# SamsungLabs/cloud_transformers

Hardware: AMD Instinct MI355X
Metric: points/sec fwd+bwd MHCT, 4096-pt batch, 1/2/4/8 MI355X; % HBM roofline (higher is better)
Workload: dtype f32; 1 GPU; north-star op-level: B=8 clouds x N=4096 pts, H=64 heads, C=16 feat/head, 2D grid W=32, reduce=max, keys=tanh(randn), seed 1234+rank; step = Splat fwd, Slice fwd, Slice bwd, Splat bwd (key cotangents summed); per_gpu_batch=8, parallelism=replica-sharded clouds x1 (no collective), world_size_seen=1, hip_graph=True, steps_per_graph=10

## Files before the change

### cloud_transformers_amd/csrc/ct_raster_bwd_fused.h

```cpp
#pragma once

template <bool HAS_PAD, int WT, int NT = 0, int CT = 0>
__global__ void __launch_bounds__(kSortThreads) slice_splat_bwd_kernel(RasterArgs a_arg, GridW<2> g_arg) {
  const GridW<2> g = grid2_of<WT>(g_arg);
  RasterArgs a = a_arg;
  if constexpr (NT > 0) a.N = NT;
  if constexpr (CT > 0) a.C = CT;
  extern __shared__ __align__(16) unsigned char lds_raw[];
  const int G = WT ? WT * WT : g.G, W1 = WT ? WT : g.W[1], N = a.N, C = a.C;
  const SortLds L = sort_lds(G, N, C);
  float4* T4 = (float4*)(lds_raw + L.tile);
  int* acc = (int*)(lds_raw + L.acc);
  float4* ZG = (float4*)(lds_raw + L.tile);
  float4* Sg = (float4*)(lds_raw + L.stage);
  const float2* AB = (const float2*)(lds_raw + L.ab);
  unsigned* s_max = (unsigned*)(lds_raw + L.misc);
  unsigned* s_k = s_max + C;
  int* s_tie = (int*)(s_k + 1);
  const int b = blockIdx.z;
  const size_t bh = (size_t)b * a.H + blockIdx.y;
  const int tid = threadIdx.x;
  const int off[4] = {0, W1, 1, W1 + 1};
  const bool has = (tid << 2) < N;
  const int n0 = has ? (tid << 2) : 0;
  const int ngroups = C >> 2;
  const float* const feat = a.tile_in2;

  float gq[4][4];
  float fq[4][4];
  float cvq[4];
  const float* const src0 = a.src + bh * C * (size_t)N;
  const float* const fea0 = feat + bh * C * (size_t)N;
  const float* const cnv0 = a.tile_in + bh * C * (size_t)G;
  const unsigned ln0 = (unsigned)n0, lc0 = (unsigned)(tid < G ? tid : 0);
  auto request1 = [&](int grp, int cj) {
    const float4 t = ld_stream4(src0 + (size_t)(grp * 4 + cj) * N + ln0);
    gq[cj][0] = t.x; gq[cj][1] = t.y; gq[cj][2] = t.z; gq[cj][3] = t.w;
    cvq[cj] = ld_stream(cnv0 + (size_t)(grp * 4 + cj) * G + lc0);
  };
  auto request_feat1 = [&](int grp, int cj) {
    const float4 t = ld_stream4(fea0 + (size_t)(grp * 4 + cj) * N + ln0);
    fq[cj][0] = t.x; fq[cj][1] = t.y; fq[cj][2] = t.z; fq[cj][3] = t.w;
  };
  PlaneKeys PK;
  load_plane_keys(a, g, W1, bh, PK);
  SortedPlane S;
  float pv[4];
#pragma unroll
  for (int i = 0; i < 4; ++i) pv[i] = (HAS_PAD && has) ? ct_load_pad(a.pad, a.pad_dtype, (size_t)b * N + n0 + i) : 1.0f;

  sort_plane(a, PK, G, W1, sort_ptrs(lds_raw, L, C), C, S, nullptr, [&]() {
#pragma unroll
    for (int cj = 0; cj < 4; ++cj) request1(0, cj);
  });
  for (int i = tid; i < G; i += kSortThreads) ((int4*)acc)[i] = make_int4(0, 0, 0, 0);
  if (tid == 0) Sg[N] = make_float4(0.0f, 0.0f, 0.0f, 0.0f);
  if (tid < 4) s_tie[tid] = 0;
  const float Kf = (float)(*s_k);

  float gsx[2][kItemLen], gsy[2][kItemLen];
#pragma unroll
  for (int u = 0; u < 2; ++u)
#pragma unroll
    for (int j = 0; j < kItemLen; ++j) gsx[u][j] = gsy[u][j] = 0.0f;
  float gs[4][2];
#pragma unroll
  for (int i = 0; i < 4; ++i) gs[i][0] = gs[i][1] = 0.0f;
  unsigned long long tied = 0ull;

  const float* const key0 = a.pos.keys + bh * 2 * (size_t)N;

  auto group = [&](const int grp, auto more) {
    const int ch0 = grp * 4;
    asm volatile("" : "+v"(S.rk01), "+v"(S.rk23));
#pragma unroll
    for (int cj = 0; cj < 4; ++cj) {
      float m = 0.0f;
#pragma unroll
      for (int i = 0; i < 4; ++i) {
        float x = HAS_PAD ? gq[cj][i] * pv[i] : gq[cj][i];
        x = has ? x : 0.0f;
        gq[cj][i] = x;
        x = fabsf(x);
        m = fmaxf(m, (x < __builtin_inff()) ? x : __builtin_inff());
      }
      const unsigned mb = wave_max_u32(__float_as_uint(m));
      if ((tid & 63) == 0) atomicMax(&s_max[ch0 + cj], mb);
    }
    if (has) {
      const unsigned rk[4] = {S.rk01 & kRankMask, (S.rk01 >> 16) & kRankMask, S.rk23 & kRankMask, (S.rk23 >> 16) & kRankMask};
#pragma unroll
      for (int i = 0; i < 4; ++i) Sg[rk[i]] = make_float4(gq[0][i], gq[1][i], gq[2][i], gq[3][i]);
    }
    if (tid < G) T4[tid] = make_float4(cvq[0], cvq[1], cvq[2], cvq[3]);
    __syncthreads();

    float iq[4];
    bool any_float = false;
#pragma unroll
    for (int cj = 0; cj < 4; ++cj) {
      float q;
      bool fixed;
      fx_quantum(__uint_as_float(s_max[ch0 + cj]) * Kf, q, iq[cj], fixed);
      if (!fixed) {
        iq[cj] = 0.0f;
        any_float = true;
      }
      iq[cj] = __uint_as_float(__builtin_amdgcn_readfirstlane(__float_as_uint(iq[cj])));
    }
    auto item = [&](auto U) {
      constexpr int u = decltype(U)::value;
      const int Y = S.cell[u] < 0 ? 0 : S.cell[u];
      asm volatile("" : "+v"(S.ent8[u][0]), "+v"(S.ent8[u][1]));
      float4 cv[4];
#pragma unroll
      for (int v = 0; v < 4; ++v) cv[v] = T4[Y + off[v]];
      float4 xn = *(const float4*)((const unsigned char*)Sg + 2u * CT_E8(S, u, 0));
      float2 wn = *(const float2*)((const unsigned char*)AB + CT_E8(S, u, 0));
      ct_f2 s01[4], s23[4];
#pragma unroll
      for (int v = 0; v < 4; ++v) s01[v] = s23[v] = ct_f2{0.0f, 0.0f};
#pragma unroll
      for (int j = 0; j < kItemLen; ++j) {
        if constexpr (u == 0) request_feat1(grp, j);
        const float4 x = xn;
        const float2 wf = wn;
        if (j + 1 < kItemLen) {
          xn = *(const float4*)((const unsigned char*)Sg + 2u * CT_E8(S, u, j + 1));
          wn = *(const float2*)((const unsigned char*)AB + CT_E8(S, u, j + 1));
        }
        const ct_f2 x01 = {x.x, x.y}, x23 = {x.z, x.w};
        const float w1x = wf.x, w1y = wf.y, w0x = 1.0f - w1x, w0y = 1.0f - w1y;
        const float cw[4] = {w0x * w0y, w1x * w0y, w0x * w1y, w1x * w1y};
        float gw[4];
#pragma unroll
        for (int v = 0; v < 4; ++v) {
          const ct_f2 cwv = {cw[v], cw[v]};
          s01[v] = __builtin_elementwise_fma(x01, cwv, s01[v]);
          s23[v] = __builtin_elementwise_fma(x23, cwv, s23[v]);
          const ct_f2 c01 = {cv[v].x, cv[v].y}, c23 = {cv[v].z, cv[v].w};
          const ct_f2 pr = __builtin_elementwise_fma(c23, x23, c01 * x01);
          gw[v] = pr.x + pr.y;
        }
        gsx[u][j] = __builtin_fmaf(gw[3] - gw[2], w1y, __builtin_fmaf(gw[1] - gw[0], w0y, gsx[u][j]));
        gsy[u][j] = __builtin_fmaf(gw[3] - gw[1], w1x, __builtin_fmaf(gw[2] - gw[0], w0x, gsy[u][j]));
        asm volatile("" : "+v"(gsx[u][j]), "+v"(gsy[u][j]));
        CT_SB;
      }
      if (S.cell[u] >= 0) {
        const ct_f2 iq01 = {iq[0], iq[1]}, iq23 = {iq[2], iq[3]};
        int* Tc = acc + Y;
#pragma unroll
        for (int v = 0; v < 4; ++v) {
          const ct_f2 a01 = s01[v] * iq01, a23 = s23[v] * iq23;
          atomicAdd(Tc + off[v], cvt_rpi(a01.x));
          atomicAdd(Tc + G + off[v], cvt_rpi(a01.y));
          atomicAdd(Tc + 2 * G + off[v], cvt_rpi(a23.x));
          atomicAdd(Tc + 3 * G + off[v], cvt_rpi(a23.y));
        }
      }
      CT_SB;
    };
    item(std::integral_constant<int, 0>{});
    if (S.cell[1] >= 0) item(std::integral_constant<int, 1>{});
    if (any_float) {
#pragma unroll 1
      for (int cj = 0; cj < 4; ++cj)
        if (iq[cj] == 0.0f) scatter_float_channel<HAS_PAD>(a, g, bh, b, ch0 + cj, (float*)(acc + cj * G), 1, 0);
    }
    const float4 tx = *(const float4*)(key0 + ln0), ty = *(const float4*)(key0 + N + ln0);
    __syncthreads();

    float4 zc = make_float4(0.0f, 0.0f, 0.0f, 0.0f);
    float gv[4] = {0.0f, 0.0f, 0.0f, 0.0f};
    if (tid < G) {
      zc = T4[tid];
      float* gout = a.tile_out + (bh * C + ch0) * (size_t)G + tid;
#pragma unroll
      for (int cj = 0; cj < 4; ++cj) {
        float q, iqd;
        bool fixed;
        fx_quantum(__uint_as_float(s_max[ch0 + cj]) * Kf, q, iqd, fixed);
        const int r = acc[cj * G + tid];
        gv[cj] = fixed ? (float)r * q : __int_as_float(r);
        __builtin_nontemporal_store(gv[cj], gout + (size_t)cj * G);
      }
    }
    const unsigned zw[4] = {__float_as_uint(zc.x), __float_as_uint(zc.y), __float_as_uint(zc.z), __float_as_uint(zc.w)};
    {
      int nzt = 0;
#pragma unroll
      for (int k = 0; k < 4; ++k) nzt += (zw[k] != 0u);
      nzt = wave_sum_i32(nzt);
      if ((tid & 63) == 0 && nzt) atomicAdd(&s_tie[(grp & 1) * 2], nzt);
    }
    __syncthreads();
    if (tid < G) {
      ZG[tid] = make_float4(__uint_as_float(zw[0] ? zw[0] : kNoMatch), __uint_as_float(zw[1] ? zw[1] : kNoMatch), gv[0], gv[1]);
      ZG[G + tid] = make_float4(__uint_as_float(zw[2] ? zw[2] : kNoMatch), __uint_as_float(zw[3] ? zw[3] : kNoMatch), gv[2], gv[3]);
    }
    __syncthreads();

    int nm = 0;
    if (has) {
      float kx[4] = {tx.x, tx.y, tx.z, tx.w}, ky[4] = {ty.x, ty.y, ty.z, ty.w};
#pragma unroll
      for (int i = 0; i < 4; ++i) {
        if constexpr (decltype(more)::value) request1(grp + 1, i);
        asm volatile("" : "+v"(kx[i]), "+v"(ky[i]));
        Pt2 p;
        pt2_from_keys(kx[i], ky[i], g, W1, p);
        float gw[4] = {0.0f, 0.0f, 0.0f, 0.0f};
#pragma unroll
        for (int pr = 0; pr < 2; ++pr) {
          const float4* Zp = ZG + (size_t)pr * G + p.base;
          const float xa = HAS_PAD ? fq[2 * pr][i] * pv[i] : fq[2 * pr][i];
          const float xb = HAS_PAD ? fq[2 * pr + 1][i] * pv[i] : fq[2 * pr + 1][i];
          ct_f4 zg[4];
#pragma unroll
          for (int v = 0; v < 4; ++v) zg[v] = *(const ct_f4*)(Zp + off[v]);
#pragma unroll
          for (int v = 0; v < 4; ++v) asm volatile("" : "+v"(zg[v].x), "+v"(zg[v].y), "+v"(zg[v].z), "+v"(zg[v].w));
          float gfa = 0.0f, gfb = 0.0f;
#pragma unroll
          for (int v = 0; v < 4; ++v) {
            const unsigned ba = __float_as_uint(xa * p.cw[v]), bb = __float_as_uint(xb * p.cw[v]);
            const bool ma = ba == __float_as_uint(zg[v].x), mb = bb == __float_as_uint(zg[v].y);
            nm += (int)ma;
            nm += (int)mb;
            asm volatile("" : "+v"(nm));
            const float ga = ma ? zg[v].z : 0.0f, gb = mb ? zg[v].w : 0.0f;
            gfa = __builtin_fmaf(ga, p.cw[v], gfa);
            gfb = __builtin_fmaf(gb, p.cw[v], gfb);
            gw[v] = __builtin_fmaf(gb, xb, __builtin_fmaf(ga, xa, gw[v]));
          }
          fq[2 * pr][i] = HAS_PAD ? gfa * pv[i] : gfa;
          fq[2 * pr + 1][i] = HAS_PAD ? gfb * pv[i] : gfb;
        }
        gs[i][0] = __builtin_fmaf(gw[3] - gw[2], p.w1y, __builtin_fmaf(gw[1] - gw[0], p.w0y, gs[i][0]));
        gs[i][1] = __builtin_fmaf(gw[3] - gw[1], p.w1x, __builtin_fmaf(gw[2] - gw[0], p.w0x, gs[i][1]));
        asm volatile("" : "+v"(gs[i][0]), "+v"(gs[i][1]), "+v"(fq[0][i]), "+v"(fq[1][i]), "+v"(fq[2][i]), "+v"(fq[3][i]));
        __builtin_amdgcn_sched_barrier(0);
      }
#pragma unroll
      for (int cj = 0; cj < 4; ++cj)
        st_stream4(a.dst + (bh * C + ch0 + cj) * (size_t)N + n0, make_float4(fq[cj][0], fq[cj][1], fq[cj][2], fq[cj][3]));
    } else if constexpr (decltype(more)::value) {
#pragma unroll
      for (int cj = 0; cj < 4; ++cj) request1(grp + 1, cj);
    }
    nm = wave_sum_i32(nm);
    if ((tid & 63) == 0 && nm) atomicAdd(&s_tie[(grp & 1) * 2 + 1], nm);
    __syncthreads();
    const int* tw = s_tie + (grp & 1) * 2;
    if (tw[0] != tw[1]) tied |= 1ull << grp;
    if (tid < 2) s_tie[((grp & 1) ^ 1) * 2 + tid] = 0;
    if (tid < G) ((int4*)acc)[tid] = make_int4(0, 0, 0, 0);
  };
  int grp = 0;
  for (; grp + 1 < ngroups; ++grp) group(grp, std::true_type{});
  group(grp, std::false_type{});

  if (tied != 0ull) {
    __builtin_amdgcn_fence(__ATOMIC_RELEASE, "workgroup");
    asm volatile("s_waitcnt vmcnt(0)" ::: "memory");
    __syncthreads();
    __builtin_amdgcn_fence(__ATOMIC_ACQUIRE, "workgroup");
    RasterArgs a2 = a;
    a2.src = feat;
    PtRows R;
    R.Nr = N; R.so = 0; R.wt = false;
    for (int gi = 0; gi < ngroups; ++gi) {
      if (!((tied >> gi) & 1ull)) continue;
      const int cabs = gi << 2;
      const float* zin = a.tile_in + (bh * C + cabs) * (size_t)G;
      const float* gin = a.tile_out + (bh * C + cabs) * (size_t)G;
      __syncthreads();
      {
        int nz_unused = 0;
        unsigned long long nzp_unused = 0ull;
        unsigned xzp_unused = 0u;
        stage_tile_pairs<false>(ZG, zin, gin, 2, G, nz_unused, nzp_unused, xzp_unused);
      }
      __syncthreads();
      if (has) {
        const float4 tx = *(const float4*)(key0 + ln0), ty = *(const float4*)(key0 + N + ln0);
        const float kx[4] = {tx.x, tx.y, tx.z, tx.w}, ky[4] = {ty.x, ty.y, ty.z, ty.w};
        int nm_unused = 0;
        unsigned u0 = 0u, u1 = 0u;
        splat_bwd_quad<HAS_PAD, true, WT, true>(a2, g, ZG, bh, b, cabs, 4, n0, R, kx, ky, gs, nm_unused, u0, u1, false);
      }
    }
    __syncthreads();
  }

  float2* Gs = (float2*)Sg;
#pragma unroll
  for (int u = 0; u < 2; ++u)
#pragma unroll
    for (int j = 0; j < kItemLen; ++j)
      *(float2*)((unsigned char*)Gs + CT_E8(S, u, j)) = make_float2(gsx[u][j], gsy[u][j]);
  __syncthreads();
  if (has) {
    const unsigned rw[4] = {S.rk01 & 0xffffu, S.rk01 >> 16, S.rk23 & 0xffffu, S.rk23 >> 16};
    float2 gk[4];
#pragma unroll
    for (int i = 0; i < 4; ++i) {
      gk[i] = Gs[rw[i] & kRankMask];
      gk[i].x *= (rw[i] & kInsideX) ? 1.0f : 0.0f;
      gk[i].y *= (rw[i] & kInsideY) ? 1.0f : 0.0f;
    }
    if (a.fold_gpos != nullptr) {
      st_stream4(a.fold_gpos + (bh * 2 + 0) * N + n0, make_float4(gk[0].x, gk[1].x, gk[2].x, gk[3].x));
      st_stream4(a.fold_gpos + (bh * 2 + 1) * N + n0, make_float4(gk[0].y, gk[1].y, gk[2].y, gk[3].y));
    }
    const float4 tx = *(const float4*)(key0 + ln0), ty = *(const float4*)(key0 + N + ln0);
    float4 ox = make_float4(gs[0][0] * ct_key_mask(tx.x), gs[1][0] * ct_key_mask(tx.y), gs[2][0] * ct_key_mask(tx.z), gs[3][0] * ct_key_mask(tx.w));
    float4 oy = make_float4(gs[0][1] * ct_key_mask(ty.x), gs[1][1] * ct_key_mask(ty.y), gs[2][1] * ct_key_mask(ty.z), gs[3][1] * ct_key_mask(ty.w));
    ox.x += gk[0].x; ox.y += gk[1].x; ox.z += gk[2].x; ox.w += gk[3].x;
    oy.x += gk[0].y; oy.y += gk[1].y; oy.z += gk[2].y; oy.w += gk[3].y;
    *(float4*)(a.g_pos + (bh * 2 + 0) * N + n0) = ox;
    *(float4*)(a.g_pos + (bh * 2 + 1) * N + n0) = oy;
  }
}
```

Measured before the change: 193.9 million points/s.

## Use buffer-resource streaming loads and reuse sorted-plane weights instead of reloading keys

Replaces the global streaming loads and stores of point, cell and feature rows with raw buffer loads and stores that use a per-block resource descriptor and scalar row offsets. This is meant to cut 64-bit address arithmetic and VGPR use. The per-group reload of point keys and the pt2_from_keys recomputation are replaced by reading bilinear weights from the sorted AB LDS table plus base cells stashed in LDS. The final key mask comes from the inside bits in the rank words rather than a key reload. This trades global key traffic and ALU work for extra LDS reads, and it assumes the per-plane data fits in 32-bit buffer offsets.

```diff
diff --git a/cloud_transformers_amd/csrc/ct_raster_bwd_fused.h b/cloud_transformers_amd/csrc/ct_raster_bwd_fused.h
--- a/cloud_transformers_amd/csrc/ct_raster_bwd_fused.h
+++ b/cloud_transformers_amd/csrc/ct_raster_bwd_fused.h
@@ -1,4 +1,29 @@
 #pragma once
+
+typedef unsigned ct_u4 __attribute__((ext_vector_type(4)));
+struct StreamBuf {
+  __amdgpu_buffer_rsrc_t r;
+};
+constexpr int kBufNt = 2;
+__device__ __forceinline__ StreamBuf stream_buf(const float* base, unsigned bytes) {
+  StreamBuf b;
+  b.r = __builtin_amdgcn_make_buffer_rsrc((void*)base, 0, (int)bytes, 0x00020000);
+  return b;
+}
+__device__ __forceinline__ float4 buf_ld_stream4(const StreamBuf& b, unsigned voff, unsigned soff) {
+  const ct_u4 v = __builtin_amdgcn_raw_buffer_load_b128(b.r, (int)voff, (int)soff, kBufNt);
+  return make_float4(__uint_as_float(v.x), __uint_as_float(v.y), __uint_as_float(v.z), __uint_as_float(v.w));
+}
+__device__ __forceinline__ float buf_ld_stream(const StreamBuf& b, unsigned voff, unsigned soff) {
+  return __uint_as_float(__builtin_amdgcn_raw_buffer_load_b32(b.r, (int)voff, (int)soff, kBufNt));
+}
+__device__ __forceinline__ void buf_st_stream4(const StreamBuf& b, unsigned voff, unsigned soff, float4 v) {
+  const ct_u4 t = {__float_as_uint(v.x), __float_as_uint(v.y), __float_as_uint(v.z), __float_as_uint(v.w)};
+  __builtin_amdgcn_raw_buffer_store_b128(t, b.r, (int)voff, (int)soff, kBufNt);
+}
+__device__ __forceinline__ void buf_st_stream(const StreamBuf& b, unsigned voff, unsigned soff, float v) {
+  __builtin_amdgcn_raw_buffer_store_b32(__float_as_uint(v), b.r, (int)voff, (int)soff, kBufNt);
+}
 
 template <bool HAS_PAD, int WT, int NT = 0, int CT = 0>
 __global__ void __launch_bounds__(kSortThreads) slice_splat_bwd_kernel(RasterArgs a_arg, GridW<2> g_arg) {
@@ -29,17 +54,21 @@
   float gq[4][4];
   float fq[4][4];
   float cvq[4];
-  const float* const src0 = a.src + bh * C * (size_t)N;
-  const float* const fea0 = feat + bh * C * (size_t)N;
-  const float* const cnv0 = a.tile_in + bh * C * (size_t)G;
-  const unsigned ln0 = (unsigned)n0, lc0 = (unsigned)(tid < G ? tid : 0);
+  const unsigned ln0 = (unsigned)n0;
+  const unsigned pt_row = (unsigned)N * 4u, cell_row = (unsigned)G * 4u;
+  const StreamBuf b_src = stream_buf(a.src + bh * C * (size_t)N, (unsigned)C * pt_row);
+  const StreamBuf b_fea = stream_buf(feat + bh * C * (size_t)N, (unsigned)C * pt_row);
+  const StreamBuf b_dst = stream_buf(a.dst + bh * C * (size_t)N, (unsigned)C * pt_row);
+  const StreamBuf b_cnv = stream_buf(a.tile_in + bh * C * (size_t)G, (unsigned)C * cell_row);
+  const StreamBuf b_gz = stream_buf(a.tile_out + bh * C * (size_t)G, (unsigned)C * cell_row);
+  const unsigned vo_pt = ln0 * 4u, vo_cell = tid < G ? (unsigned)tid * 4u : 0u;
   auto request1 = [&](int grp, int cj) {
-    const float4 t = ld_stream4(src0 + (size_t)(grp * 4 + cj) * N + ln0);
+    const float4 t = buf_ld_stream4(b_src, vo_pt, (unsigned)(grp * 4 + cj) * pt_row);
     gq[cj][0] = t.x; gq[cj][1] = t.y; gq[cj][2] = t.z; gq[cj][3] = t.w;
-    cvq[cj] = ld_stream(cnv0 + (size_t)(grp * 4 + cj) * G + lc0);
+    cvq[cj] = buf_ld_stream(b_cnv, vo_cell, (unsigned)(grp * 4 + cj) * cell_row);
   };
   auto request_feat1 = [&](int grp, int cj) {
-    const float4 t = ld_stream4(fea0 + (size_t)(grp * 4 + cj) * N + ln0);
+    const float4 t = buf_ld_stream4(b_fea, vo_pt, (unsigned)(grp * 4 + cj) * pt_row);
     fq[cj][0] = t.x; fq[cj][1] = t.y; fq[cj][2] = t.z; fq[cj][3] = t.w;
   };
   PlaneKeys PK;
@@ -53,6 +82,8 @@
 #pragma unroll
     for (int cj = 0; cj < 4; ++cj) request1(0, cj);
   });
+  uint2* const s_cell = (uint2*)(lds_raw + L.mark);
+  s_cell[tid] = make_uint2((unsigned)PK.base[0] | (unsigned)PK.base[1] << 16, (unsigned)PK.base[2] | (unsigned)PK.base[3] << 16);
   for (int i = tid; i < G; i += kSortThreads) ((int4*)acc)[i] = make_int4(0, 0, 0, 0);
   if (tid == 0) Sg[N] = make_float4(0.0f, 0.0f, 0.0f, 0.0f);
   if (tid < 4) s_tie[tid] = 0;
@@ -66,13 +97,13 @@
   float gs[4][2];
 #pragma unroll
   for (int i = 0; i < 4; ++i) gs[i][0] = gs[i][1] = 0.0f;
+  unsigned cell01 = ((unsigned)S.cell[0] & 0xffffu) | (unsigned)S.cell[1] << 16;
   unsigned long long tied = 0ull;
-
-  const float* const key0 = a.pos.keys + bh * 2 * (size_t)N;
 
   auto group = [&](const int grp, auto more) {
     const int ch0 = grp * 4;
-    asm volatile("" : "+v"(S.rk01), "+v"(S.rk23));
+    asm volatile("" : "+v"(S.rk01), "+v"(S.rk23), "+v"(cell01));
+    const int cell[2] = {(int)(short)(cell01 & 0xffffu), (int)cell01 >> 16};
 #pragma unroll
     for (int cj = 0; cj < 4; ++cj) {
       float m = 0.0f;
@@ -110,8 +141,8 @@
     }
     auto item = [&](auto U) {
       constexpr int u = decltype(U)::value;
-      const int Y = S.cell[u] < 0 ? 0 : S.cell[u];
-      asm volatile("" : "+v"(S.ent8[u][0]), "+v"(S.ent8[u][1]));
+      int Y = cell[u] < 0 ? 0 : cell[u];
+      asm volatile("" : "+v"(S.ent8[u][0]), "+v"(S.ent8[u][1]), "+v"(Y));
       float4 cv[4];
 #pragma unroll
       for (int v = 0; v < 4; ++v) cv[v] = T4[Y + off[v]];
@@ -147,7 +178,7 @@
         asm volatile("" : "+v"(gsx[u][j]), "+v"(gsy[u][j]));
         CT_SB;
       }
-      if (S.cell[u] >= 0) {
+      if (cell[u] >= 0) {
         const ct_f2 iq01 = {iq[0], iq[1]}, iq23 = {iq[2], iq[3]};
         int* Tc = acc + Y;
 #pragma unroll
@@ -162,20 +193,18 @@
       CT_SB;
     };
     item(std::integral_constant<int, 0>{});
-    if (S.cell[1] >= 0) item(std::integral_constant<int, 1>{});
+    if (cell[1] >= 0) item(std::integral_constant<int, 1>{});
     if (any_float) {
 #pragma unroll 1
       for (int cj = 0; cj < 4; ++cj)
         if (iq[cj] == 0.0f) scatter_float_channel<HAS_PAD>(a, g, bh, b, ch0 + cj, (float*)(acc + cj * G), 1, 0);
     }
-    const float4 tx = *(const float4*)(key0 + ln0), ty = *(const float4*)(key0 + N + ln0);
     __syncthreads();
 
     float4 zc = make_float4(0.0f, 0.0f, 0.0f, 0.0f);
     float gv[4] = {0.0f, 0.0f, 0.0f, 0.0f};
     if (tid < G) {
       zc = T4[tid];
-      float* gout = a.tile_out + (bh * C + ch0) * (size_t)G + tid;
 #pragma unroll
       for (int cj = 0; cj < 4; ++cj) {
         float q, iqd;
@@ -183,7 +212,7 @@
         fx_quantum(__uint_as_float(s_max[ch0 + cj]) * Kf, q, iqd, fixed);
         const int r = acc[cj * G + tid];
         gv[cj] = fixed ? (float)r * q : __int_as_float(r);
-        __builtin_nontemporal_store(gv[cj], gout + (size_t)cj * G);
+        buf_st_stream(b_gz, vo_cell, (unsigned)(ch0 + cj) * cell_row, gv[cj]);
       }
     }
     const unsigned zw[4] = {__float_as_uint(zc.x), __float_as_uint(zc.y), __float_as_uint(zc.z), __float_as_uint(zc.w)};
@@ -203,13 +232,17 @@
 
     int nm = 0;
     if (has) {
-      float kx[4] = {tx.x, tx.y, tx.z, tx.w}, ky[4] = {ty.x, ty.y, ty.z, ty.w};
+      const uint2 bc = s_cell[tid];
+      const unsigned rk[4] = {S.rk01 & kRankMask, (S.rk01 >> 16) & kRankMask, S.rk23 & kRankMask, (S.rk23 >> 16) & kRankMask};
+      const int pbase[4] = {(int)(bc.x & 0xffffu), (int)(bc.x >> 16), (int)(bc.y & 0xffffu), (int)(bc.y >> 16)};
 #pragma unroll
       for (int i = 0; i < 4; ++i) {
         if constexpr (decltype(more)::value) request1(grp + 1, i);
-        asm volatile("" : "+v"(kx[i]), "+v"(ky[i]));
+        const float2 w1 = AB[rk[i]];
         Pt2 p;
-        pt2_from_keys(kx[i], ky[i], g, W1, p);
+        p.w1x = w1.x; p.w1y = w1.y; p.w0x = 1.0f - w1.x; p.w0y = 1.0f - w1.y;
+        p.base = pbase[i];
+        p.cw[0] = p.w0x * p.w0y; p.cw[1] = p.w1x * p.w0y; p.cw[2] = p.w0x * p.w1y; p.cw[3] = p.w1x * p.w1y;
         float gw[4] = {0.0f, 0.0f, 0.0f, 0.0f};
 #pragma unroll
         for (int pr = 0; pr < 2; ++pr) {
@@ -244,7 +277,7 @@
       }
 #pragma unroll
       for (int cj = 0; cj < 4; ++cj)
-        st_stream4(a.dst + (bh * C + ch0 + cj) * (size_t)N + n0, make_float4(fq[cj][0], fq[cj][1], fq[cj][2], fq[cj][3]));
+        buf_st_stream4(b_dst, vo_pt, (unsigned)(ch0 + cj) * pt_row, make_float4(fq[cj][0], fq[cj][1], fq[cj][2], fq[cj][3]));
     } else if constexpr (decltype(more)::value) {
 #pragma unroll
       for (int cj = 0; cj < 4; ++cj) request1(grp + 1, cj);
@@ -255,7 +288,9 @@
     const int* tw = s_tie + (grp & 1) * 2;
     if (tw[0] != tw[1]) tied |= 1ull << grp;
     if (tid < 2) s_tie[((grp & 1) ^ 1) * 2 + tid] = 0;
-    if (tid < G) ((int4*)acc)[tid] = make_int4(0, 0, 0, 0);
+    int zero;
+    asm volatile("v_mov_b32 %0, 0" : "=v"(zero));
+    if (tid < G) ((int4*)acc)[tid] = make_int4(zero, zero, zero, zero);
   };
   int grp = 0;
   for (; grp + 1 < ngroups; ++grp) group(grp, std::true_type{});
@@ -284,6 +319,7 @@
       }
       __syncthreads();
       if (has) {
+        const float* const key0 = a.pos.keys + bh * 2 * (size_t)N;
         const float4 tx = *(const float4*)(key0 + ln0), ty = *(const float4*)(key0 + N + ln0);
         const float kx[4] = {tx.x, tx.y, tx.z, tx.w}, ky[4] = {ty.x, ty.y, ty.z, ty.w};
         int nm_unused = 0;
@@ -314,9 +350,14 @@
       st_stream4(a.fold_gpos + (bh * 2 + 0) * N + n0, make_float4(gk[0].x, gk[1].x, gk[2].x, gk[3].x));
       st_stream4(a.fold_gpos + (bh * 2 + 1) * N + n0, make_float4(gk[0].y, gk[1].y, gk[2].y, gk[3].y));
     }
-    const float4 tx = *(const float4*)(key0 + ln0), ty = *(const float4*)(key0 + N + ln0);
-    float4 ox = make_float4(gs[0][0] * ct_key_mask(tx.x), gs[1][0] * ct_key_mask(tx.y), gs[2][0] * ct_key_mask(tx.z), gs[3][0] * ct_key_mask(tx.w));
-    float4 oy = make_float4(gs[0][1] * ct_key_mask(ty.x), gs[1][1] * ct_key_mask(ty.y), gs[2][1] * ct_key_mask(ty.z), gs[3][1] * ct_key_mask(ty.w));
+    float mx[4], my[4];
+#pragma unroll
+    for (int i = 0; i < 4; ++i) {
+      mx[i] = (rw[i] & kInsideX) ? 1.0f : 0.0f;
+      my[i] = (rw[i] & kInsideY) ? 1.0f : 0.0f;
+    }
+    float4 ox = make_float4(gs[0][0] * mx[0], gs[1][0] * mx[1], gs[2][0] * mx[2], gs[3][0] * mx[3]);
+    float4 oy = make_float4(gs[0][1] * my[0], gs[1][1] * my[1], gs[2][1] * my[2], gs[3][1] * my[3]);
     ox.x += gk[0].x; ox.y += gk[1].x; ox.z += gk[2].x; ox.w += gk[3].x;
     oy.x += gk[0].y; oy.y += gk[1].y; oy.z += gk[2].y; oy.w += gk[3].y;
     *(float4*)(a.g_pos + (bh * 2 + 0) * N + n0) = ox;
```

New measurement: 211.3 million points/s (median of 6 runs). 1.09x the previous value.
